# tanqiu98/2G-GCN

Measured on AMD Instinct MI355X. Metric: clips/sec fwd+bwd, T=120 N=34 C=512, higher is better.
Workload: dtype fp32

## Files before the change

2g-gcn_amd/csrc/gemm_f32.hip:

```cpp
#include <cstdlib>
#include "twog_common.h"

typedef float f32x16 __attribute__((ext_vector_type(16)));
typedef float f32x4 __attribute__((ext_vector_type(4)));

namespace {

constexpr int BK = 32;
constexpr int MAXP = 8;

struct Prob {
    twog_rows_t A, B, C;
    const float* bias;
    int M, N, K;
    int act, accumulate;
    int tiles_m, tiles_n, tile_start;
    int a_vec, b_vec;
    int n_major;
    int batch;
    int64_t a_bs, b_bs, c_bs;
    float* cs;
    int cs_acc;
};

// ... 1278 lines not shown
__global__ __launch_bounds__(256, 2) void gemm_ks32_kernel(const Group g) {
    gemm_tile<32, 64, 256, false, BKM, D, false, false, 2>(g, nullptr);
}
template <int D>
__global__ __launch_bounds__(256, 2) void gemm_gate_bwd_ks32_kernel(const Group g, const GateArgs ga) {
    gemm_tile<32, 64, 256, false, true, D, false, true, 2>(g, &ga);
}

template <int BM, int BN>
__global__ __launch_bounds__(256) void splitk_reduce_kernel(const Group g) {
    int bid = blockIdx.x;
    int pi = 0;
#pragma unroll 1
    for (int i = 1; i < g.n; ++i)
        if (bid >= g.p[i].tile_start) pi = i;
    const Prob& P = g.p[pi];
    int tile = bid - P.tile_start;
    const int per_batch = P.tiles_m * P.tiles_n, bi = tile / per_batch;
    tile -= bi * per_batch;
    twog_rows_t C = P.C;
    C.ptr += bi * P.c_bs;
    int tm_idx, tn_idx;
    tile_coords(P, tile, g.group, tm_idx, tn_idx);
    const int m0 = tm_idx * BM, n0 = tn_idx * BN;
    if (P.cs && tn_idx == 0 && blockIdx.y == gridDim.y - 1 && threadIdx.x < 128 && m0 + (int)threadIdx.x < P.M) {
        float v = 0.f;
        for (int s = 0; s < g.splitk; ++s) v += g.cs_part[((int64_t)s * g.total_tiles + bid) * 128 + threadIdx.x];
        float* o = P.cs + m0 + threadIdx.x;
        *o = P.cs_acc ? *o + v : v;
    }
    const int chunk = (BM * BN) / gridDim.y;
    const bool vec = (P.N % 4 == 0) && (reinterpret_cast<uintptr_t>(C.ptr) % 16 == 0) && (C.ld_outer % 4 == 0) &&
                     (C.inner <= 1 || C.ld_inner % 4 == 0) && (!P.bias || reinterpret_cast<uintptr_t>(P.bias) % 16 == 0);
    if (vec) {
        for (int e = blockIdx.y * chunk + threadIdx.x * 4; e < (blockIdx.y + 1) * chunk; e += 1024) {
            const int row = e / BN, col = e - row * BN;
            if (m0 + row >= P.M || n0 + col >= P.N) continue;
            f32x4 v = {0.f, 0.f, 0.f, 0.f};
            for (int s = 0; s < g.splitk; ++s)
                v += *reinterpret_cast<const f32x4*>(g.slabs + ((int64_t)s * g.total_tiles + bid) * (BM * BN) + e);
            float* c = C.ptr + twog_row_off(C, m0 + row) + n0 + col;
            if (P.bias) v += *reinterpret_cast<const f32x4*>(P.bias + n0 + col);
            if (P.accumulate) v += *reinterpret_cast<const f32x4*>(c);
            if (P.act == 1) { v.x = fmaxf(v.x, 0.f); v.y = fmaxf(v.y, 0.f); v.z = fmaxf(v.z, 0.f); v.w = fmaxf(v.w, 0.f); }
            *reinterpret_cast<f32x4*>(c) = v;
        }
        return;
    }
    for (int e = blockIdx.y * chunk + threadIdx.x; e < (blockIdx.y + 1) * chunk; e += 256) {
        const int row = e / BN, col = e - row * BN;
        if (m0 + row >= P.M || n0 + col >= P.N) continue;
        float v = 0.f;
        for (int s = 0; s < g.splitk; ++s) v += g.slabs[((int64_t)s * g.total_tiles + bid) * (BM * BN) + e];
        float* c = C.ptr + twog_row_off(C, m0 + row) + n0 + col;
        if (P.bias) v += P.bias[n0 + col];
        if (P.accumulate) v += *c;
        if (P.act == 1) v = fmaxf(v, 0.f);
        *c = v;
    }
}

inline int vec_ok(const twog_rows_t& m, int64_t batch_stride, int contiguous_extent, int64_t n_rows) {
    const int64_t groups = m.inner > 1 ? (n_rows + m.inner - 1) / m.inner : n_rows;
    const int64_t extent = groups * (m.ld_outer < 0 ? -m.ld_outer : m.ld_outer) + (m.inner > 1 ? (int64_t)m.inner * m.ld_inner : 0);
    if (extent >= (int64_t(1) << 30)) return 0;
    const bool aligned = (reinterpret_cast<uintptr_t>(m.ptr) % 16) == 0;
    const bool ld_ok = (m.ld_outer % 4 == 0) && (m.inner <= 1 || m.ld_inner % 4 == 0) && (batch_stride % 4 == 0);
    return (aligned && ld_ok && contiguous_extent >= 4 && contiguous_extent % 4 == 0) ? 1 : 0;
}

thread_local int g_last_class_x3 = 0;
thread_local int g_precision = TWOG_GEMM_PRECISION_HIGHEST;

template <int NP>
static void launch_x3_128(const Group& g, bool akm, bool bkm, bool kg, dim3 grid, dim3 block, hipStream_t st) {
    if (!akm && !bkm) hipLaunchKernelGGL((gemm_x3_kernel<false, false, false, NP>), grid, block, 0, st, g);
    else if (!akm && bkm && !kg) hipLaunchKernelGGL((gemm_x3_kernel<false, true, false, NP>), grid, block, 0, st, g);
    else if (!akm && bkm) hipLaunchKernelGGL((gemm_x3_kernel<false, true, true, NP>), grid, block, 0, st, g);
    else if (akm && bkm && !kg) hipLaunchKernelGGL((gemm_x3_kernel<true, true, false, NP>), grid, block, 0, st, g);
    else if (akm && bkm) hipLaunchKernelGGL((gemm_x3_kernel<true, true, true, NP>), grid, block, 0, st, g);
    else if (!kg) hipLaunchKernelGGL((gemm_x3_kernel<true, false, false, NP>), grid, block, 0, st, g);
    else hipLaunchKernelGGL((gemm_x3_kernel<true, false, true, NP>), grid, block, 0, st, g);
}

static bool x3_128_ok(const Group& g) {
    static const int x3_on = getenv("TWOG_GEMM_X3") ? atoi(getenv("TWOG_GEMM_X3")) : 1;
    bool ok = x3_on != 0 && (g.k_per_split % X3_BK) == 0;
    for (int i = 0; i < g.n; ++i) ok = ok && g.p[i].a_vec && g.p[i].b_vec && (g.p[i].K % X3_BK) == 0 && g.p[i].M >= 4 && g.p[i].N >= 4;
    return ok;
}

template <int BM, int BN, int NT, int D>
int launch(Group& g, int akm, int bkm, hipStream_t st) {
    g_last_class_x3 = 0;
    dim3 grid(g.total_tiles, g.splitk), block(NT);
    bool kg = false;
    for (int i = 0; i < g.n; ++i) kg = kg || (akm && g.p[i].A.inner > 1) || (bkm && g.p[i].B.inner > 1);
    if constexpr (BM == 128 && NT == 512) {
        if (x3_128_ok(g)) {
            static const int split_acc = getenv("TWOG_X3_DW_SPLIT_ACC") ? atoi(getenv("TWOG_X3_DW_SPLIT_ACC")) : 0;
            const int np = (akm && bkm && split_acc) ? 3 : g_precision == TWOG_GEMM_PRECISION_HIGH ? 2 : g_precision == TWOG_GEMM_PRECISION_MEDIUM ? 1 : 3;
            if (np == 2) launch_x3_128<2>(g, akm, bkm, kg, grid, block, st);
            else if (np == 1) launch_x3_128<1>(g, akm, bkm, kg, grid, block, st);
            else if (!akm && !bkm) hipLaunchKernelGGL((gemm_x3_kernel<false, false, false>), grid, block, 0, st, g);
            else if (!akm && bkm && !kg) hipLaunchKernelGGL((gemm_x3_kernel<false, true, false>), grid, block, 0, st, g);
            else if (!akm && bkm) hipLaunchKernelGGL((gemm_x3_kernel<false, true, true>), grid, block, 0, st, g);
            else if (akm && bkm && split_acc && !kg) hipLaunchKernelGGL((gemm_x3_tt_split_acc_kernel<false>), grid, block, 0, st, g);
            else if (akm && bkm && split_acc) hipLaunchKernelGGL((gemm_x3_tt_split_acc_kernel<true>), grid, block, 0, st, g);
            else if (akm && bkm && !kg) hipLaunchKernelGGL((gemm_x3_kernel<true, true, false>), grid, block, 0, st, g);
            else if (akm && bkm) hipLaunchKernelGGL((gemm_x3_kernel<true, true, true>), grid, block, 0, st, g);
            else if (!kg) hipLaunchKernelGGL((gemm_x3_kernel<true, false, false>), grid, block, 0, st, g);
            else hipLaunchKernelGGL((gemm_x3_kernel<true, false, true>), grid, block, 0, st, g);
            TWOG_CHECK_LAUNCH();
            g_last_class_x3 = np;
            if (g.splitk > 1) {
                hipLaunchKernelGGL((splitk_reduce_kernel<BM, BN>), dim3(g.total_tiles, (BM * BN) / 1024), dim3(256), 0, st, g);
                TWOG_CHECK_LAUNCH();
            }
            return 0;
        }
        if (kg) return launch<BM, BN, 256, D>(g, akm, bkm, st);
    }
    if (!akm && !bkm) hipLaunchKernelGGL((gemm_kernel<BM, BN, NT, false, false, D, false>), grid, block, 0, st, g);
    else if (!akm && bkm && !kg) hipLaunchKernelGGL((gemm_kernel<BM, BN, NT, false, true, D, false>), grid, block, 0, st, g);
    else if (!akm && bkm) hipLaunchKernelGGL((gemm_kernel<BM, BN, NT, false, true, D, true>), grid, block, 0, st, g);
    else if (akm && bkm && !kg) hipLaunchKernelGGL((gemm_kernel<BM, BN, NT, true, true, D, false>), grid, block, 0, st, g);
    else if (akm && bkm) hipLaunchKernelGGL((gemm_kernel<BM, BN, NT, true, true, D, true>), grid, block, 0, st, g);
    else if (!kg) hipLaunchKernelGGL((gemm_kernel<BM, BN, NT, true, false, D, false>), grid, block, 0, st, g);
    else hipLaunchKernelGGL((gemm_kernel<BM, BN, NT, true, false, D, true>), grid, block, 0, st, g);
    TWOG_CHECK_LAUNCH();
    if (g.splitk > 1) {
        hipLaunchKernelGGL((splitk_reduce_kernel<BM, BN>), dim3(g.total_tiles, (BM * BN) / 1024), dim3(256), 0, st, g);
        TWOG_CHECK_LAUNCH();
    }
    return 0;
}

thread_local int g_last_class = 0;

}

extern "C" int twog_gemm_last_class(void) { return g_last_class; }

extern "C" int twog_gemm_set_precision(int p) {
    if (p != TWOG_GEMM_PRECISION_HIGHEST && p != TWOG_GEMM_PRECISION_HIGH && p != TWOG_GEMM_PRECISION_MEDIUM) return -1;
    const int prev = g_precision;
    g_precision = p;
    return prev;
}
extern "C" int twog_gemm_get_precision(void) { return g_precision; }

constexpr size_t SPLITK_TICKET_BYTES = 16384;

static void prepare_group(const twog_gemm_t* pr, int n, int a_kmajor, int b_kmajor, void* workspace,
                          size_t workspace_bytes, Group& g, int* order, bool& big, int& bm) {
    int64_t tiles128 = 0;
    int kmax = 0;
    bool wide = true;
    for (int i = 0; i < n; ++i) {
        const int nb = pr[i].batch > 0 ? pr[i].batch : 1;
        tiles128 += (int64_t)nb * ((pr[i].M + 127) / 128) * ((pr[i].N + 127) / 128);
        if (pr[i].K > kmax) kmax = pr[i].K;
        if (pr[i].M < 96 || pr[i].N < 96) wide = false;
    }
    static const int force_tile = getenv("TWOG_GEMM_TILE") ? atoi(getenv("TWOG_GEMM_TILE")) : 0;
    static const int force_split = getenv("TWOG_GEMM_SPLITK") ? atoi(getenv("TWOG_GEMM_SPLITK")) : 0;
    const int64_t reach128 = tiles128 * (workspace ? (kmax >= 1024 ? kmax / 512 : 1) : 1);
    static const int big_min = getenv("TWOG_GEMM_BIG_MIN") ? atoi(getenv("TWOG_GEMM_BIG_MIN")) : 200;
    big = wide && (tiles128 >= big_min || reach128 >= 256);
    if (force_tile == 128) big = true;
    if (force_tile == 64) big = false;
    const int BMN = big ? 128 : 64;
    bm = BMN;
    {
        static const int bm32_on = getenv("TWOG_GEMM_BM32") ? atoi(getenv("TWOG_GEMM_BM32")) : 1;
        static const int ks_allowed = getenv("TWOG_GEMM_KS") ? atoi(getenv("TWOG_GEMM_KS")) : 1;
        int64_t tiles32 = 0;
        bool plain = true;
        for (int i = 0; i < n; ++i) {
            tiles32 += (int64_t)((pr[i].M + 31) / 32) * ((pr[i].N + 63) / 64);
            plain = plain && pr[i].batch <= 1 && !(b_kmajor && pr[i].B.inner > 1);
        }
        if (bm32_on && ks_allowed && !big && !a_kmajor && !workspace && plain && kmax >= 256 && tiles32 <= 256) bm = 32;
    }
    g.n = n;
    for (int i = 0; i < n; ++i) order[i] = i;
    for (int i = 1; i < n; ++i)
        for (int j = i; j > 0 && pr[order[j]].K > pr[order[j - 1]].K; --j) { const int tmp = order[j]; order[j] = order[j - 1]; order[j - 1] = tmp; }
    int t = 0;
    g.n_cls = 0;
    for (int i = 0; i < n; ++i) {
        Prob& P = g.p[i];
        const twog_gemm_t& q = pr[order[i]];
        P.A = q.A; P.B = q.B; P.C = q.C; P.bias = q.bias;
        P.M = q.M; P.N = q.N; P.K = q.K;
        P.act = q.act; P.accumulate = q.accumulate;
        P.cs = q.a_colsum; P.cs_acc = q.a_colsum_accumulate;
        P.tiles_m = (P.M + bm - 1) / bm;
        P.tiles_n = (P.N + BMN - 1) / BMN;
        P.tile_start = t;
        P.batch = q.batch > 0 ? q.batch : 1;
        static const int force_nmajor = getenv("TWOG_GEMM_NMAJOR") ? atoi(getenv("TWOG_GEMM_NMAJOR")) : -1;
        P.n_major = force_nmajor >= 0 ? force_nmajor : (P.N > P.M ? 1 : 0);
        P.a_bs = q.a_batch_stride; P.b_bs = q.b_batch_stride; P.c_bs = q.c_batch_stride;
        const int ntiles = P.batch * P.tiles_m * P.tiles_n;
        if (i == 0 || P.K != g.p[i - 1].K) {
            g.cls_start[g.n_cls] = t;
            g.cls_ntiles[g.n_cls] = 0;
            ++g.n_cls;
        }
        g.cls_ntiles[g.n_cls - 1] += ntiles;
        t += ntiles;
        P.a_vec = vec_ok(P.A, q.a_batch_stride, a_kmajor ? P.M : P.K, a_kmajor ? P.K : P.M);
        P.b_vec = vec_ok(P.B, q.b_batch_stride, b_kmajor ? P.N : P.K, b_kmajor ? P.K : P.N);
    }
    for (int c = 0, rot = 0; c < g.n_cls; ++c) {
        g.cls_rot[c] = rot & 7;
        rot += g.cls_ntiles[c] & 7;
    }
    g.total_tiles = t;
    static const int group = getenv("TWOG_GEMM_GROUP") ? atoi(getenv("TWOG_GEMM_GROUP")) : 8;
    static const int group64 = getenv("TWOG_GEMM_GROUP64") ? atoi(getenv("TWOG_GEMM_GROUP64")) : 0;
    g.group = big ? group : group64;
    g.splitk = 1;
    g.k_per_split = ((kmax + BK - 1) / BK) * BK;
    g.slabs = nullptr;
    g.cs_part = nullptr;
    g.xcnt = nullptr;
    g.xs_early = 0;
    g.xcd_split = 0;
    if (t < 4096 && kmax >= 1024 && workspace) {
        const int slots = big ? 512 : 1024;
        const int max_by_k = kmax / 256;
        int want = 1;
        double best = 0.0;
        const int max_split = t < 384 ? 64 : 16;
        for (int sft = 1; sft <= max_split && sft <= max_by_k; ++sft) {
            const int64_t wg = (int64_t)t * sft;
            if (wg > (t < 384 ? 2 : 8) * slots && sft > 1) break;
            const double eff = (double)wg / (double)(((wg + slots - 1) / slots) * slots);
            if (eff > best + 0.03) { best = eff; want = sft; }
        }
        if (force_split > 0) want = force_split;
        static const int xcd_on = getenv("TWOG_GEMM_XCD_SPLIT") ? atoi(getenv("TWOG_GEMM_XCD_SPLIT")) : 1;
        int want8 = 0;
        if (xcd_on && big && want > 1 && force_split <= 0 && t <= 512) {
            double best8 = 0.0;
            for (int s8 = 8; s8 <= 64 && s8 <= kmax / 1024; s8 += 8) {
                if ((size_t)s8 * t * BMN * BMN * sizeof(float) + SPLITK_TICKET_BYTES > workspace_bytes) break;
                const int64_t per_xcd = (int64_t)t * s8 / 8;
                const double e8 = (double)per_xcd / (double)(((per_xcd + 63) / 64) * 64);
                if (e8 > best8 + 1e-9) { best8 = e8; want8 = s8; }
                if (e8 >= 0.95) break;
            }
            if (want8 && best8 + 0.08 < best) want8 = 0;
        }
        if (want8) want = want8;
        bool any_cs = false;
        for (int i = 0; i < n; ++i) any_cs = any_cs || pr[i].a_colsum != nullptr;
        const size_t cs_bytes = any_cs ? (size_t)(want + 1) * t * 128 * sizeof(float) : 0;
        const size_t need = (size_t)want * t * BMN * BMN * sizeof(float) + SPLITK_TICKET_BYTES + cs_bytes;
        if (want > 1 && need <= workspace_bytes) {
            int kps = (kmax + want - 1) / want;
            g.k_per_split = ((kps + BK - 1) / BK) * BK;
            g.splitk = (kmax + g.k_per_split - 1) / g.k_per_split;
            g.slabs = reinterpret_cast<float*>(static_cast<char*>(workspace) + SPLITK_TICKET_BYTES);
            g.xcd_split = (want8 && g.splitk % 8 == 0) ? 1 : 0;
            if (any_cs) g.cs_part = g.slabs + (size_t)g.splitk * t * BMN * BMN;
        }
    }
}

static bool x3s_ok(const Group& g, int a_kmajor, int xk, int min_tiles = 96) {
    static const int on = (getenv("TWOG_GEMM_X3") ? atoi(getenv("TWOG_GEMM_X3")) : 1) && (getenv("TWOG_GEMM_X3S") ? atoi(getenv("TWOG_GEMM_X3S")) : 1);
    if (!on || a_kmajor || g.splitk != 1 || g.total_tiles < min_tiles) return false;
    int kmax = 0;
    for (int i = 0; i < g.n; ++i) {
        const Prob& P = g.p[i];
        if (!P.a_vec || !P.b_vec || P.K % xk || P.batch > 1 || P.B.inner > 1 || P.M < 1 || P.N < 4) return false;
        kmax = P.K > kmax ? P.K : kmax;
    }
    return kmax >= 256;
}

static int x3s_ku(const Group& g, int depth) {
    static const int ku = getenv("TWOG_X3S_KU") ? atoi(getenv("TWOG_X3S_KU")) : 2;
    if (ku <= 1) return 1;
    for (int i = 0; i < g.n; ++i)
        if (g.p[i].K % depth) return 1;
    return ku;
}

constexpr size_t XS_COUNTER_BYTES = 16384;
static int pick_xsplit(int tiles, int kmax, int bm, size_t ws_bytes) {
    static const int force = getenv("TWOG_GEMM_XSPLIT") ? atoi(getenv("TWOG_GEMM_XSPLIT")) : 0;
    if (force == 1 || tiles <= 0 || tiles > 4096 || ws_bytes <= XS_COUNTER_BYTES) return 1;
    const int kt = (kmax + BK - 1) / BK;
    const size_t tile_bytes = (size_t)bm * 64 * sizeof(float);
    const int by_ws = (int)((ws_bytes - XS_COUNTER_BYTES) / (tile_bytes * (size_t)tiles));
    if (bm == 32 && force <= 1) {
        int S = kt / 4 < 8 ? kt / 4 : 8;
        while (S > 1 && (tiles * S > 512 || S > by_ws)) --S;
        return S < 1 ? 1 : S;
    }
    const double unit = bm == 32 ? 0.25 : 0.49;
    auto cost = [&](int S) {
        const int per_cu = (tiles * S + 255) / 256, kts = (kt + S - 1) / S;
        return per_cu * kts * unit + (S > 1 ? 3.0 + 0.35 * S : 0.0);
    };
    int best = 1;
    double best_c = cost(1);
    static const int cand[] = {2, 3, 4, 6, 8, 12, 16};
    for (int S : cand) {
        if (S > by_ws || kt / S < 2) break;
        const double c = force > 1 ? (S == force ? -1.0 : 1e30) : cost(S);
        if (c < best_c - 2.5) { best_c = c; best = S; }
    }
    return best;
}

template <class LaunchFn>
static bool try_xsplit(Group& g, int bm, int kmax, void* chain_ws, size_t chain_ws_bytes, LaunchFn launch_fn) {
    if (!chain_ws) return false;
    const int S = pick_xsplit(g.total_tiles, kmax, bm, chain_ws_bytes);
    if (S <= 1) return false;
    const int kt = (kmax + BK - 1) / BK;
    g.k_per_split = ((kt + S - 1) / S) * BK;
    g.splitk = (kmax + g.k_per_split - 1) / g.k_per_split;
    if (g.splitk <= 1) { g.splitk = 1; g.k_per_split = kt * BK; return false; }
    g.xcnt = reinterpret_cast<unsigned*>(chain_ws);
    g.slabs = reinterpret_cast<float*>(reinterpret_cast<char*>(chain_ws) + XS_COUNTER_BYTES);
    static const int early_tiles = getenv("TWOG_GEMM_XS_EARLY") ? atoi(getenv("TWOG_GEMM_XS_EARLY")) : 96;
    g.xs_early = g.total_tiles <= early_tiles ? 1 : 0;
    launch_fn(dim3(g.total_tiles, g.splitk));
    return true;
}

static int pick_xl_split(int tiles, int kmax, size_t ws_bytes) {
    static const int force = getenv("TWOG_X3_XL") ? atoi(getenv("TWOG_X3_XL")) : 0;
    if (force == 1 || tiles < 96 || tiles > 4096 || ws_bytes <= XS_COUNTER_BYTES || kmax % 32) return 1;
    const int kt = kmax / 32;
    const int by_ws = (int)((ws_bytes - XS_COUNTER_BYTES) / ((size_t)64 * 64 * sizeof(float) * (size_t)tiles));
    auto cost = [&](int S) {
        const int r = (tiles * S + 255) / 256;
        return r * ((kt + S - 1) / S) + (S > 1 ? 3 + r : 0);
    };
    int best = 1;
    int best_c = cost(1);
    static const int min_gain = getenv("TWOG_X3_XL_GAIN") ? atoi(getenv("TWOG_X3_XL_GAIN")) : 15;
    static const int cand[] = {2, 3, 4};
    for (int S : cand) {
        if (S > by_ws || kt / S < 8) break;
        const int c = force > 1 ? (S == force ? -1 : (1 << 20)) : cost(S);
        if (c * 100 <= best_c * (100 - min_gain)) { best_c = c; best = S; }
    }
    return best;
}
static bool xl_setup(Group& g, int kmax, void* chain_ws, size_t chain_ws_bytes) {
    if (!chain_ws) return false;
    const int S = pick_xl_split(g.total_tiles, kmax, chain_ws_bytes);
    if (S <= 1) return false;
    const int kt = kmax / 32;
    g.k_per_split = ((kt + S - 1) / S) * 32;
    g.splitk = (kmax + g.k_per_split - 1) / g.k_per_split;
    if (g.splitk <= 1) { g.splitk = 1; g.k_per_split = ((kmax + BK - 1) / BK) * BK; return false; }
    g.xcnt = reinterpret_cast<unsigned*>(chain_ws);
    g.slabs = reinterpret_cast<float*>(reinterpret_cast<char*>(chain_ws) + XS_COUNTER_BYTES);
    g.xcd_split = 0;
    return true;
}

static bool colsums_served(const twog_gemm_t* pr, int n, int a_kmajor, int b_kmajor, const Group& g, bool big) {
    bool any = false, plain = true;
    for (int i = 0; i < n; ++i) {
        any = any || pr[i].a_colsum != nullptr;
        plain = plain && pr[i].batch <= 1 && pr[i].M % 4 == 0 && pr[i].A.inner <= 1 && pr[i].B.inner <= 1;
    }
    if (!any) return true;
    static const int w8 = getenv("TWOG_GEMM_W8") ? atoi(getenv("TWOG_GEMM_W8")) : 1;
    return a_kmajor && b_kmajor && big && w8 && plain && x3_128_ok(g);
}

static bool rows128_pays(const Group& g) {
    static const int on = getenv("TWOG_X3_ROWS128") ? atoi(getenv("TWOG_X3_ROWS128")) : 1;
    if (!on) return false;
    int t64 = 0, t128 = 0;
    for (int i = 0; i < g.n; ++i) {
        const Prob& P = g.p[i];
        if (P.M < 128 || P.batch > 1) return false;
        t64 += ((P.M + 63) / 64) * P.tiles_n;
        t128 += ((P.M + 127) / 128) * P.tiles_n;
    }
    if (t128 < 128 || t128 > 256) return false;
    const int c64 = ((t64 + 255) / 256) * 128, c128 = ((t128 + 255) / 256) * 192;
    return c128 * 100 <= c64 * 85;
}
static void retile_rows(Group& g, int bm) {
    int t = 0;
    g.n_cls = 0;
    for (int i = 0; i < g.n; ++i) {
        Prob& P = g.p[i];
        P.tiles_m = (P.M + bm - 1) / bm;
        P.tile_start = t;
        const int ntiles = P.batch * P.tiles_m * P.tiles_n;
        if (i == 0 || P.K != g.p[i - 1].K) {
            g.cls_start[g.n_cls] = t;
            g.cls_ntiles[g.n_cls] = 0;
            ++g.n_cls;
        }
        g.cls_ntiles[g.n_cls - 1] += ntiles;
        t += ntiles;
    }
    for (int c = 0, rot = 0; c < g.n_cls; ++c) {
        g.cls_rot[c] = rot & 7;
        rot += g.cls_ntiles[c] & 7;
    }
    g.total_tiles = t;
}

static int gemm_impl(const twog_gemm_t* problems, int n_problems, int a_kmajor, int b_kmajor, void* workspace,
                     size_t workspace_bytes, void* chain_ws, size_t chain_ws_bytes, void* stream);

extern "C" int twog_gemm_colsum_fused(const twog_gemm_t* problems, int n_problems, int a_kmajor, int b_kmajor, void* workspace,
                                      size_t workspace_bytes) {
    for (int done = 0; done < n_problems; done += MAXP) {
        const int n = (n_problems - done) < MAXP ? (n_problems - done) : MAXP;
        Group g;
        int order[MAXP];
        bool big;
        int bm;
        prepare_group(problems + done, n, a_kmajor, b_kmajor, workspace, workspace_bytes, g, order, big, bm);
        if (!colsums_served(problems + done, n, a_kmajor, b_kmajor, g, big)) return 0;
    }
    return 1;
}

extern "C" int twog_gemm_f32(const twog_gemm_t* problems, int n_problems, int a_kmajor, int b_kmajor, void* workspace,
                             size_t workspace_bytes, void* stream) {
    return gemm_impl(problems, n_problems, a_kmajor, b_kmajor, workspace, workspace_bytes, nullptr, 0, stream);
}

extern "C" int twog_gemm_f32_chain(const twog_gemm_t* problems, int n_problems, int a_kmajor, int b_kmajor, void* chain_ws,
                                   size_t chain_ws_bytes, void* stream) {
    return gemm_impl(problems, n_problems, a_kmajor, b_kmajor, nullptr, 0, chain_ws, chain_ws_bytes, stream);
}

extern "C" size_t twog_chain_workspace_bytes(void) {
    return XS_COUNTER_BYTES + (size_t)48 * 1024 * 1024;
}

static int gemm_impl(const twog_gemm_t* problems, int n_problems, int a_kmajor, int b_kmajor, void* workspace,
                     size_t workspace_bytes, void* chain_ws, size_t chain_ws_bytes, void* stream) {
    if (n_problems <= 0) return 0;
    hipStream_t st = reinterpret_cast<hipStream_t>(stream);
    {
        bool any_cs = false;
        for (int i = 0; i < n_problems; ++i) any_cs = any_cs || problems[i].a_colsum != nullptr;
        if (any_cs && (chain_ws || !twog_gemm_colsum_fused(problems, n_problems, a_kmajor, b_kmajor, workspace, workspace_bytes))) return -5;
    }
    int done = 0;
    while (done < n_problems) {
        const int n = (n_problems - done) < MAXP ? (n_problems - done) : MAXP;
        const twog_gemm_t* pr = problems + done;
        Group g;
        int order[MAXP];
        bool big;
        int bm;
        prepare_group(pr, n, a_kmajor, b_kmajor, workspace, workspace_bytes, g, order, big, bm);
        static const int depth = getenv("TWOG_GEMM_DEPTH") ? atoi(getenv("TWOG_GEMM_DEPTH")) : 0;
        const int d128 = depth ? (depth & 3) : 2, d64 = depth ? ((depth >> 2) & 3) : 2;
        int rc;
        static const int w8 = getenv("TWOG_GEMM_W8") ? atoi(getenv("TWOG_GEMM_W8")) : 1;
        bool grouped = false;
        for (int i = 0; i < n; ++i) grouped = grouped || (a_kmajor && pr[i].A.inner > 1) || (b_kmajor && pr[i].B.inner > 1);
        g_last_class = (big ? TWOG_GEMM_CLASS_TILE128 : 0) | (big && w8 && !grouped ? TWOG_GEMM_CLASS_WAVES8 : 0) |
                       (grouped ? TWOG_GEMM_CLASS_KG : 0) | (g.splitk > 1 ? TWOG_GEMM_CLASS_SPLITK : 0);
        static const int ks_on = getenv("TWOG_GEMM_KS") ? atoi(getenv("TWOG_GEMM_KS")) : 1;
        int kmax_ = 0;
        for (int i = 0; i < n; ++i) kmax_ = pr[i].K > kmax_ ? pr[i].K : kmax_;
        const bool ks = ks_on && !big && !a_kmajor && !grouped && g.splitk == 1 && g.total_tiles <= 384 && kmax_ >= 256;
        if (!big && bm == 64 && !grouped && chain_ws && x3s_ok(g, a_kmajor, 32) && rows128_pays(g)) {
            retile_rows(g, 128);
            g_last_class |= TWOG_GEMM_CLASS_X3 | TWOG_GEMM_CLASS_WAVES8;
            dim3 grid(g.total_tiles, 1), block(512);
            if (b_kmajor) hipLaunchKernelGGL((gemm_x3su128_kernel<true>), grid, block, 0, st, g);
            else hipLaunchKernelGGL((gemm_x3su128_kernel<false>), grid, block, 0, st, g);
            TWOG_CHECK_LAUNCH();
            done += n;
            continue;
        }
        if (!big && bm == 64 && !grouped && chain_ws && x3s_ok(g, a_kmajor, 32) && xl_setup(g, kmax_, chain_ws, chain_ws_bytes)) {
            g_last_class |= TWOG_GEMM_CLASS_X3 | TWOG_GEMM_CLASS_XSPLIT;
            dim3 grid(g.total_tiles, g.splitk), block(256);
            if (b_kmajor) hipLaunchKernelGGL((gemm_x3su_kernel<true, 1, 2>), grid, block, 0, st, g);
            else hipLaunchKernelGGL((gemm_x3su_kernel<false, 1, 2>), grid, block, 0, st, g);
            TWOG_CHECK_LAUNCH();
            done += n;
            continue;
        }
        if (bm == 32) {
            g_last_class |= TWOG_GEMM_CLASS_KSPLIT | TWOG_GEMM_CLASS_ROWS32;
            if (try_xsplit(g, 32, kmax_, chain_ws, chain_ws_bytes, [&](dim3 grid) {
                    if (b_kmajor) hipLaunchKernelGGL((gemm_xs32_kernel<true, 2>), grid, dim3(256), 0, st, g);
                    else hipLaunchKernelGGL((gemm_xs32_kernel<false, 2>), grid, dim3(256), 0, st, g);
                })) {
                g_last_class |= TWOG_GEMM_CLASS_XSPLIT;
                TWOG_CHECK_LAUNCH();
                done += n;
                continue;
            }
            dim3 grid(g.total_tiles, 1), block(256);
            if (b_kmajor) hipLaunchKernelGGL((gemm_ks32_kernel<true, 2>), grid, block, 0, st, g);
            else hipLaunchKernelGGL((gemm_ks32_kernel<false, 2>), grid, block, 0, st, g);
            TWOG_CHECK_LAUNCH();
            done += n;
            continue;
        }
        if (ks) {
            g_last_class |= TWOG_GEMM_CLASS_KSPLIT;
            if (try_xsplit(g, 64, kmax_, chain_ws, chain_ws_bytes, [&](dim3 grid) {
                    if (b_kmajor) hipLaunchKernelGGL((gemm_xs_kernel<true, 2>), grid, dim3(512), 0, st, g);
                    else hipLaunchKernelGGL((gemm_xs_kernel<false, 2>), grid, dim3(512), 0, st, g);
                })) {
                g_last_class |= TWOG_GEMM_CLASS_XSPLIT;
                TWOG_CHECK_LAUNCH();
                done += n;
                continue;
            }
            dim3 grid(g.total_tiles, 1), block(512);
            if (x3s_ok(g, a_kmajor, 32)) {
                g_last_class |= TWOG_GEMM_CLASS_X3;
                if (g.total_tiles <= 256 && x3s_ku(g, 64) == 2) {
                    if (b_kmajor) hipLaunchKernelGGL((gemm_x3su_kernel<true, 2, 2>), grid, block, 0, st, g);
                    else hipLaunchKernelGGL((gemm_x3su_kernel<false, 2, 2>), grid, block, 0, st, g);
                } else if (b_kmajor) hipLaunchKernelGGL((gemm_x3s_kernel<true, 2>), grid, block, 0, st, g);
                else hipLaunchKernelGGL((gemm_x3s_kernel<false, 2>), grid, block, 0, st, g);
            } else if (b_kmajor) hipLaunchKernelGGL((gemm_ks_kernel<true, 2>), grid, block, 0, st, g);
            else hipLaunchKernelGGL((gemm_ks_kernel<false, 2>), grid, block, 0, st, g);
            TWOG_CHECK_LAUNCH();
            done += n;
            continue;
        }
        static const int x3_try = getenv("TWOG_GEMM_X3") ? atoi(getenv("TWOG_GEMM_X3")) : 1;
        if (big && w8 && (!grouped || x3_try)) rc = d128 == 2 ? launch<128, 128, 512, 2>(g, a_kmajor, b_kmajor, st) : launch<128, 128, 512, 1>(g, a_kmajor, b_kmajor, st);
        else if (big) rc = d128 == 2 ? launch<128, 128, 256, 2>(g, a_kmajor, b_kmajor, st) : launch<128, 128, 256, 1>(g, a_kmajor, b_kmajor, st);
        else if (!big && x3s_ok(g, a_kmajor, 16)) {
            g_last_class |= TWOG_GEMM_CLASS_X3;
            dim3 grid(g.total_tiles, 1), block(256);
            if (x3s_ku(g, 32) == 2) {
                if (b_kmajor) hipLaunchKernelGGL((gemm_x3su_kernel<true, 1, 2>), grid, block, 0, st, g);
                else hipLaunchKernelGGL((gemm_x3su_kernel<false, 1, 2>), grid, block, 0, st, g);
            } else if (b_kmajor) hipLaunchKernelGGL((gemm_x3s_kernel<true, 1>), grid, block, 0, st, g);
            else hipLaunchKernelGGL((gemm_x3s_kernel<false, 1>), grid, block, 0, st, g);
            TWOG_CHECK_LAUNCH();
            rc = 0;
        }
        else rc = d64 == 2 ? launch<64, 64, 256, 2>(g, a_kmajor, b_kmajor, st) : launch<64, 64, 256, 1>(g, a_kmajor, b_kmajor, st);
        if (rc) return rc;
        if (g_last_class_x3) g_last_class |= TWOG_GEMM_CLASS_X3 | TWOG_GEMM_CLASS_WAVES8 |
                                             (g_last_class_x3 == 2 ? TWOG_GEMM_CLASS_P3 : g_last_class_x3 == 1 ? TWOG_GEMM_CLASS_P1 : 0);
        done += n;
    }
    return 0;
}


int twog_internal_gemm_gate_bwd(const twog_gemm_t* pr, int n, const twog_gru_step_bwd_t* gates, float* const* du_part,
                                int dry_run, void* chain_ws, size_t chain_ws_bytes, void* stream) {
    if (n <= 0 || n > MAXP) return 1;
    Group g;
    int order[MAXP];
    bool big;
    int bm;
    prepare_group(pr, n, 0, 1, nullptr, 0, g, order, big, bm);
    if (big || g.splitk != 1) return 1;
    auto span31 = [](const twog_rows_t& m, int rows, int64_t width) {
        const int inner = m.inner > 1 ? m.inner : 1;
        const int64_t last = (int64_t)((rows - 1) / inner) * m.ld_outer + (int64_t)((rows - 1) % inner) * (m.inner > 1 ? m.ld_inner : 0) + width;
        return m.ld_outer >= 0 && m.ld_inner >= 0 && last < (int64_t(1) << 31);
    };
    for (int i = 0; i < n; ++i) {
        if (pr[i].B.inner > 1 || pr[i].batch > 1 || pr[i].bias || pr[i].act) return 1;
        const twog_gru_step_bwd_t& G = gates[i];
        if (G.rows <= 0) continue;
        if ((pr[i].N + 63) / 64 > 8 || G.rows != pr[i].M || G.hidden != pr[i].N || G.rows >= (1 << 22)) return 1;
        const int inner = G.dh.inner > 1 ? G.dh.inner : 1;
        auto same = [&](const twog_rows_t& m) { return (m.inner > 1 ? m.inner : 1) == inner; };
        if (!same(G.save) || !same(G.dgi) || !same(G.dgh) || (G.h_prev.ptr && !same(G.h_prev))) return 1;
        if (G.u && (G.u_inner > 1 ? G.u_inner : 1) != inner) return 1;
        if (G.dh_prev.inner > 1 || G.dh_prev.ptr != pr[i].C.ptr || G.dh_prev_accumulate) return 1;
        const int H3 = 3 * G.hidden;
        if (!span31(G.dh, G.rows, G.hidden) || !span31(G.save, G.rows, 4 * G.hidden) || !span31(G.dgi, G.rows, H3) ||
            !span31(G.dgh, G.rows, H3) || !span31(G.dh_prev, G.rows, G.hidden) ||
            (G.h_prev.ptr && !span31(G.h_prev, G.rows, G.hidden)))
            return 1;
        if (G.u && ((int64_t)((G.rows - 1) / inner) * G.u_ld_outer + (int64_t)((G.rows - 1) % inner) * G.u_ld_inner >= (int64_t(1) << 31)))
            return 1;
    }
    if (dry_run) return 0;
    GateArgs ga;
    for (int i = 0; i < n; ++i) {
        const int src = order[i];
        ga.gate_of[i] = gates[src].rows > 0 ? i : -1;
        ga.s[i] = gates[src];
        ga.du_part[i] = (gates[src].rows > 0 && gates[src].du && du_part) ? du_part[src] : nullptr;
    }
    for (int i = n; i < MAXP; ++i) { ga.gate_of[i] = -1; ga.du_part[i] = nullptr; }
    static const int depth = getenv("TWOG_GEMM_DEPTH") ? atoi(getenv("TWOG_GEMM_DEPTH")) : 0;
    const int d64 = depth ? ((depth >> 2) & 3) : 2;
    dim3 grid(g.total_tiles, 1), block(256);
    g_last_class = TWOG_GEMM_CLASS_GATE;
    static const int ks_on = getenv("TWOG_GEMM_KS") ? atoi(getenv("TWOG_GEMM_KS")) : 1;
    int kmax = 0;
    for (int i = 0; i < n; ++i) kmax = pr[i].K > kmax ? pr[i].K : kmax;
    if (bm == 64 && chain_ws && x3s_ok(g, 0, 32) && xl_setup(g, kmax, chain_ws, chain_ws_bytes)) {
        g_last_class |= TWOG_GEMM_CLASS_X3 | TWOG_GEMM_CLASS_XSPLIT;
        hipLaunchKernelGGL((gemm_gate_bwd_x3su_kernel<1, 2>), dim3(g.total_tiles, g.splitk), dim3(256), 0, (hipStream_t)stream, g, ga);
        TWOG_CHECK_LAUNCH();
        return 0;
    }
    if (bm == 32) {
// ... 127 lines not shown
```

2g-gcn_amd/ops.py:

```python
import contextlib
import math
import os
import weakref

import torch

from .kernels import get_kernels

SUPPORTED_NOTE = ("the HIP path implements every constructor configuration of the reference's TGGCN: message_type "
                  "'v1' (relational) / 'v2', message_granularity 'v1' / 'v2', aggregation 'att' / 'mp', attention_style "
                  "'v1'..'v4', distance-based attention, every gate strategy and position feature. Sender-only messages "
                  "with dot-product attention or mean pooling (every configuration shipped in the reference's "
                  "conf/models/) run on the tuned kernels (attn.hip, segrnn.hip), the other forms on the general "
                  "single-relation kernels (relation.hip)")


def _v2(t, width=None):
    return t.view(-1, t.shape[-1] if width is None else width)


class Plan:

    def __init__(self, cfg, bs, T, H, O, N, F_o, n_sub, n_aff, human_seg_given, object_seg_given):
        h = cfg['hidden_size']
# ... 119 lines not shown
            'sh': 'geometry_to_human_message_att_mlp', 'so': 'geometry_to_object_message_att_mlp'}
_REL_ENDS = {'hh': ('h', 'h'), 'oh': ('h', 'o'), 'sh': ('h', 's'), 'ho': ('o', 'h'), 'so': ('o', 's'), 'oo': ('o', 'o')}


def _head_name(plan, name):
    return name.replace('_frame', '') if plan.share_heads else name


def used_parameter_names(plan: Plan):
    g = 'geometry_embedding_gcn.'
    names = [g + 'joint_embed.cnn.0.bn.weight', g + 'joint_embed.cnn.0.bn.bias',
             g + 'joint_embed.cnn.1.cnn.weight', g + 'joint_embed.cnn.1.cnn.bias',
             g + 'joint_embed.cnn.3.cnn.weight', g + 'joint_embed.cnn.3.cnn.bias',
             g + 'get_s.s1.cnn.weight', g + 'get_s.s1.cnn.bias', g + 'get_s.s2.cnn.weight', g + 'get_s.s2.cnn.bias',
             g + 'weight']
    for m in ('geometry_embedding_mlp.0', 'geometry_embedding_mlp.2', 'human_embedding_mlp.0',
              'object_embedding_mlp.0', 'human_bd_embedding_mlp.0', 'object_bd_embedding_mlp.0',
              'geometry_bd_embedding_mlp.0'):
        names += [m + '.weight', m + '.bias']
    for r in ('human_bd_rnn', 'object_bd_rnn', 'geometry_bd_rnn'):
        for sfx in ('', '_reverse'):
            names += [f'{r}.weight_ih_l0{sfx}', f'{r}.weight_hh_l0{sfx}', f'{r}.bias_ih_l0{sfx}', f'{r}.bias_hh_l0{sfx}']
    for rel in plan.snd_h + plan.snd_o + plan.snd_s:
        if plan.relational:
            names += [f'{_REL_PREFIX[rel]}_{kind}_relation_mlp.0.{wb}' for kind in ('pairwise', 'full')
                      for wb in ('weight', 'bias')]
        else:
            names += [_FRAME_MLP[rel] + '.0.weight', _FRAME_MLP[rel] + '.0.bias']
            if not plan.mean_pool and plan.att_style != 'dot':
                names += [_ATT_MLP[rel] + ('.weight' if plan.att_style == 'general' else '.0.weight'),
                          _ATT_MLP[rel] + ('.bias' if plan.att_style == 'general' else '.0.bias')]
    if plan.msg_segment:
        for rel in ('hh', 'ho', 'oh', 'oo'):
            if not getattr(plan, 'rel_' + rel):
                continue
            if plan.relational:
                names += [f'{_REL_PREFIX[rel]}_segment_{kind}_relation_mlp.0.{wb}' for kind in ('pairwise', 'full')
                          for wb in ('weight', 'bias')]
                continue
            names += [_SEG_MLP[rel] + '.0.weight', _SEG_MLP[rel] + '.0.bias']
            if not plan.mean_pool and plan.att_style != 'dot':
                a_ = _ATT_MLP[rel].replace('_message_att_mlp', '_segment_message_att_mlp')
                names += [a_ + ('.weight' if plan.att_style == 'general' else '.0.weight'),
                          a_ + ('.bias' if plan.att_style == 'general' else '.0.bias')]
    for cell in ('human_segment_rnn_fcell', 'human_segment_rnn_bcell', 'object_segment_rnn_fcell',
                 'object_segment_rnn_bcell'):
        names += [cell + '.weight_ih', cell + '.weight_hh', cell + '.bias_ih', cell + '.bias_hh']
    for on, mlp in ((plan.learn_h, 'update_human_segment_mlp'), (plan.own_o, 'update_object_segment_mlp')):
        if on:
            for layer in range(plan.n_gate_hidden + 1):
                names += [f'{mlp}.{2 * layer}.weight', f'{mlp}.{2 * layer}.bias']
    if not plan.periodic:
        if plan.time_s or plan.time_u:
            names += ['time_position_mlp.0.weight', 'time_position_mlp.0.bias']
        if plan.seglen:
            names += ['segment_length_mlp.0.weight', 'segment_length_mlp.0.bias']
    heads = ['human_frame_recognition_mlp', 'human_frame_prediction_mlp', 'human_recognition_mlp',
             'human_prediction_mlp']
    if plan.n_aff is not None:
        heads += ['object_frame_recognition_mlp', 'object_frame_prediction_mlp', 'object_recognition_mlp',
                  'object_prediction_mlp']
    for m in heads:
        m = _head_name(plan, m)
        names += [m + '.0.weight', m + '.0.bias']
    if not plan.has_bias:
        names = [n for n in names if n.startswith('geometry_embedding_gcn.') or
                 not (n.endswith('.bias') or '.bias_' in n)]
    seen, out = set(), []
    for n in names:
        if n not in seen:
            seen.add(n)
            out.append(n)
    return out


_MODEL_EXTRAS = weakref.WeakKeyDictionary()


def set_model_extra(model, key, value):
    d = _MODEL_EXTRAS.setdefault(model, {})
    if value is None:
        d.pop(key, None)
    else:
        d[key] = value


def get_model_extra(model, key):
    return _MODEL_EXTRAS.get(model, {}).get(key)


def set_grad_stage_hook(model, fn):
    set_model_extra(model, 'stage_hook', fn)


def pack_weights(K, groups):
    out, pairs = {}, []
    for key, tensors in groups.items():
        if not tensors:
            out[key] = None
            continue
        t0 = tensors[0]
        buf = torch.empty((sum(t.shape[0] for t in tensors),) + tuple(t0.shape[1:]), dtype=torch.float32, device=t0.device)
        r = 0
        for t in tensors:
            src = t.detach()
            pairs.append((src if src.is_contiguous() else src.contiguous(), buf[r:r + t.shape[0]]))
            r += t.shape[0]
        out[key] = buf
    K.copy_blocks(pairs)
    return out


def grad_ready_stage(name: str) -> int:
    if ('_segment_rnn_' in name or name.startswith('update_') or 'recognition_mlp' in name or 'prediction_mlp' in name
            or any(name.startswith(v) for v in _SEG_MLP.values())):
        return 0
    if '_bd_rnn' in name or '_bd_embedding_mlp' in name or any(name.startswith(v) for v in _FRAME_MLP.values()):
        return 1
    return 2


def enable_grad_sinks(params, on: bool = True):
    for p in params:
        p._twog_grad_sink = bool(on)


def _stage_done(plan, stage, G=None):
    if G is not None:
        G.flush()
    hook = getattr(plan, 'stage_hook', None)
    if isinstance(hook, weakref.WeakMethod):
        hook = hook()
    if hook is not None:
        hook(stage)


class _Params(dict):

    def __missing__(self, k):
        if k.endswith('.bias') or '.bias_' in k:
            return None
        raise KeyError(k)


class _Grads:

    def __init__(self, K, sinks=None, known=None):
        self.K, self.g, self.sinks, self.known = K, {}, sinks or {}, known
        self._pending, self._pending_dst = [], set()
        self._pend_cs, self._pend_cp = [], []
        self._pend_mm_wide = True
        self._pend_mm, self._pend_mm_c = [], set()
        self._held = None
        self._defer = hasattr(K, 'colsum_many') and os.environ.get('TWOG_BATCH_ADDS', '1') != '0'
        self._verify = os.environ.get('TWOG_VERIFY_DEFERRED', '0') == '1'
        self._snaps = []

    def _snap(self, *tensors):
        if not self._verify:
            return
        outs = [q['C'] for q in self._pend_mm] + [o for _, _, o, _ in self._pend_cs] + [d for _, d in self._pend_cp]
        if self._held is not None:
            outs += [self._held['C']] + ([self._held['colsum']] if self._held.get('colsum') is not None else [])
        pending = {o.untyped_storage().data_ptr() for o in outs}
        self._snaps += [(t, t.detach().clone()) for t in tensors
                        if t is not None and t.untyped_storage().data_ptr() not in pending]

    def _check_snaps(self):
        snaps, self._snaps = self._snaps, []
        for t, was in snaps:
            if not torch.equal(t, was):
                raise RuntimeError('an operand of a deferred gradient launch changed between the call and flush() '
                                   f'(shape {tuple(t.shape)}): the deferred form would have computed a different gradient')

    def sink(self, name):
        return self.sinks.get(name)

    def has(self, name):
        return self.known is None or dict.__contains__(self.known, name)

    def add(self, name, t):
        if not self.has(name):
            return
        dst = self.sinks.get(name)
        if dst is None:
            dst = self.g.get(name)
        if dst is not None:
            if not hasattr(self.K, 'rowops') or os.environ.get('TWOG_BATCH_ADDS', '1') == '0':
                self.K.add_rows(_v2(t.reshape(1, -1)), _v2(dst.view(1, -1)))
                return
            key = dst.data_ptr()
            if key in self._pending_dst or len(self._pending) >= 16:
                self.flush()
            self._pending.append(('add', _v2(t.reshape(1, -1)), _v2(dst.view(1, -1))))
            self._pending_dst.add(key)
            self._snap(t)
        else:
            self.g[name] = t

    def dw_gemm(self, problem):
        A, B = problem['A'], problem['B']

        def plain(t):
            n = t.shape[0] if t.dim() == 2 else t.shape[0] * t.shape[1]
            return (t.shape[-1] % 4 == 0 and t.data_ptr() % 16 == 0 and all(st % 4 == 0 for st in t.stride()[:-1]) and n % 16 == 0)

        rows = A.shape[0] if A.dim() == 2 else A.shape[0] * A.shape[1]
        wide = A.shape[-1] >= 128 and B.shape[-1] >= 128 and rows <= 8192 and plain(A) and plain(B)
        narrow = ((A.shape[-1] < 128 or B.shape[-1] < 128) and 0 < rows <= int(os.environ.get('TWOG_BATCH_DW_NARROW_ROWS', '20000')))
        if narrow and self._holdable(problem):
            narrow = False
        if not self._defer or os.environ.get('TWOG_BATCH_DW', '1') == '0' or not (wide or narrow):
            self._issue_held()
            if problem['C'].data_ptr() in self._pend_mm_c:
                self.flush()
            if self._holdable(problem):
                self._held = problem
                self._snap(A, B)
                return
            self.K.gemm([problem], a_kmajor=True, b_kmajor=True)
            return
        key = problem['C'].data_ptr()
        if key in self._pend_mm_c or len(self._pend_mm) >= 8 or (self._pend_mm and self._pend_mm_wide != wide):
            self.flush()
        self._pend_mm.append(problem)
        self._pend_mm_c.add(key)
        self._pend_mm_wide = wide
        self._snap(A, B)

    def _holdable(self, problem):
        return (self._defer and problem['A'].dim() == 2 and os.environ.get('TWOG_DW_COLSUM', '1') != '0'
                and hasattr(self.K, 'gemm_colsum_ok') and self.K.gemm_colsum_ok(problem))

    def colsum(self, x, out=None, accumulate=False):
        if out is None:
            out, accumulate = torch.empty(x.shape[-1], dtype=torch.float32, device=x.device), False
        if not self._defer:
            return self.K.colsum(x, out=out, accumulate=accumulate)
        h = self._held
        if h is not None:
            A = h['A']
            if (A.data_ptr() == x.data_ptr() and A.shape == x.shape and A.stride() == x.stride() and out.is_contiguous()
                    and not any(o.data_ptr() == out.data_ptr() for _, _, o, _ in self._pend_cs)):
                h['colsum'], h['colsum_accumulate'] = out, accumulate
            self._issue_held()
            if 'colsum' in h:
                return out
        if len(self._pend_cs) >= 16 or any(o.data_ptr() == out.data_ptr() for _, _, o, _ in self._pend_cs):
            self.flush()
        self._pend_cs.append((x, None, out, accumulate))
        self._snap(x)
        return out

    def copy(self, src, dst):
        if not self._defer:
            dst.copy_(src)
            return
        self._pend_cp.append((src, dst))

    def _issue_held(self):
        h, self._held = self._held, None
        if h is not None:
            if self._verify and not self._pend_mm and not self._pend_cs and not self._pending:
                self._check_snaps()
            self.K.gemm([h], a_kmajor=True, b_kmajor=True)

    def flush(self):
        if self._verify:
            self._check_snaps()
        self._issue_held()
        if self._pend_mm:
            self.K.gemm(self._pend_mm, a_kmajor=True, b_kmajor=True)
            self._pend_mm, self._pend_mm_c = [], set()
        if self._pend_cs:
            self.K.colsum_many(self._pend_cs)
            self._pend_cs = []
        if self._pend_cp:
            self.K.copy_blocks(self._pend_cp)
            self._pend_cp = []
        if self._pending:
            self.K.rowops(self._pending)
            self._pending, self._pending_dst = [], set()


def _gru_bias_grads(K, G, b_ih, b_hh, dgi, dgh, h):
    if not (G.has(b_ih) or G.has(b_hh)):
        return
    db_ih = G.colsum(dgi)
    if G.has(b_hh):
        db_hh = torch.empty(3 * h, dtype=torch.float32, device=dgi.device)
        G.copy(db_ih[:2 * h], db_hh[:2 * h])
        G.colsum(dgh[:, 2 * h:], out=db_hh[2 * h:])
        G.add(b_hh, db_hh)
    G.add(b_ih, db_ih)


def _lin_w_grads(K, G, wname, bname, dY, X, cols=None, total=None):
    N, Kin = dY.shape[-1], X.shape[-1]
    dst = G.sink(wname)
    if cols is not None:
        c0, c1 = cols
        if dst is None:
            dst = G.g.get(wname)
            if dst is None:
                dst = torch.zeros(N, total, dtype=torch.float32, device=dY.device)
                G.g[wname] = dst
        G.dw_gemm(dict(A=dY, B=X, C=dst.view(N, total)[:, c0:c1], accumulate=True))
    elif dst is not None:
        G.dw_gemm(dict(A=dY, B=X, C=dst.view(N, Kin), accumulate=True))
    else:
        dW = torch.empty(N, Kin, dtype=torch.float32, device=dY.device)
        G.dw_gemm(dict(A=dY, B=X, C=dW))
        G.add(wname, dW)
    _bias_grad(K, G, bname, dY)


def geo_gcn_forward(K, P, x_human, bs, T, N, training, bn_bufs, S, save_x=True):
    dev, nF = x_human.device, bs * T

    def empty(*shape):
        return torch.empty(*shape, dtype=torch.float32, device=dev)

    g = 'geometry_embedding_gcn.'
    wq, wk = P[g + 'get_s.s1.cnn.weight'].view(128, 64), P[g + 'get_s.s2.cnn.weight'].view(128, 64)
    ab, mi, md = K.bn_fold(x_human, N, P[g + 'joint_embed.cnn.0.bn.weight'], P[g + 'joint_embed.cnn.0.bn.bias'],
                           bn_bufs['running_mean'], bn_bufs['running_var'], bn_bufs['num_batches_tracked'], training,
                           stats_reduce=bn_bufs.get('stats_reduce'), fold=(wq, wk, P[g + 'get_s.s1.cnn.bias']))
    w1 = P[g + 'joint_embed.cnn.1.cnn.weight'].view(64, 4)
    w2 = P[g + 'joint_embed.cnn.3.cnn.weight'].view(64, 64)
    X, adj, Z = K.gcn_fused_fwd(x_human, N, ab, w1, P[g + 'joint_embed.cnn.1.cnn.bias'], w2,
                                P[g + 'joint_embed.cnn.3.cnn.bias'], md, save_x=save_x)
    Gout = empty(bs, 128, N, T)
    Zv = Z.view(bs, T, N, 64).permute(0, 2, 1, 3)
    K.gemm([dict(A=P[g + 'weight'], B=Zv[0], C=Gout[0].view(128, N * T), batch=(bs, 0, T * N * 64, 128 * N * T))],
           a_kmajor=True, b_kmajor=False)
    S.update(ab=ab, mi=mi, X=X, md=md, adj=adj, Z=Z)
    return Gout


def _rel_distance_view(p, dists, rel, n_inst):
    d = dists or {}
    H, O = p.H, p.O
    if rel == 'hh' and d.get('hh') is not None:
        return d['hh'].reshape(n_inst, H, H)
    if rel == 'oh' and d.get('ho') is not None:
        return d['ho'].reshape(n_inst, H, O)
    if rel == 'ho' and d.get('ho') is not None:
        return d['ho'].reshape(n_inst, H, O).transpose(1, 2)
    if rel == 'oo' and d.get('oo') is not None:
        return d['oo'].reshape(n_inst, O, O)
    return None


class _RelLevel:

    def __init__(self, p, segment, n_inst, ipc, feats, outs, dists, scale, dfeats=None, douts=None):
        self.p, self.segment, self.n_inst, self.ipc = p, segment, n_inst, ipc
        self.feats, self.outs, self.dists, self.scale = feats, outs, dists, scale
        self.dfeats, self.douts = dfeats, douts
        self.D = p.h if segment else 2 * p.h
        self.sizes = {'h': p.H, 'o': p.O, 's': 1}

    def names(self, rel):
        seg = '_segment' if self.segment else ''
        msg = (_SEG_MLP if self.segment else _FRAME_MLP)[rel] + '.0'
        att = _ATT_MLP[rel].replace('_message_att_mlp', seg + '_message_att_mlp')
        return dict(msg=msg, att=att, g=f'{_REL_PREFIX[rel]}{seg}_pairwise_relation_mlp.0',
                    f=f'{_REL_PREFIX[rel]}{seg}_full_relation_mlp.0')

    def recv_masked(self, rel):
        return (not self.segment) and rel in ('ho', 'so')


class _Staged:

    def __init__(self, K):
        self.K = K
        self._gemm, self._rf, self._rb, self._ops = {}, [], [], []

    def gemm(self, problems, **flags):
        self._gemm.setdefault(tuple(sorted(flags.items())), []).extend(problems)

    def relation_fwd(self, f):
        self._rf.append(f)

    def relation_bwd(self, b):
        self._rb.append(b)

    def relu_bwd(self, dy, y, dx):
        self._ops.append(('relu_bwd', dy, y, dx))

    def rank1_update(self, dst, s_, v):
        self._ops.append(('rank1', dst, s_, v))

    @staticmethod
    def _waves(items, targets):
        waves = []
        for it in items:
            t = targets(it)
            for w_items, w_t in waves:
                if not (t & w_t):
                    w_items.append(it)
                    w_t |= t
                    break
            else:
                waves.append(([it], set(t)))
        return [w for w, _ in waves]

    @staticmethod
    def _rb_targets(b):
        return {b[k].data_ptr() for k, acc in (('dq', 'dq_accumulate'), ('dk', 'dk_accumulate'))
                if b.get(acc) and b.get(k) is not None}

    def flush(self):
        K = self.K
        for flags, probs in self._gemm.items():
            for wave in self._waves(probs, lambda g: {g['C'].data_ptr()} if g.get('accumulate') else set()):
                K.gemm(wave, **dict(flags))
        if self._rf:
            K.relation_fwd_many(self._rf)
        for wave in self._waves(self._rb, self._rb_targets):
            K.relation_bwd_many(wave)
        for wave in self._waves(self._ops, lambda o: {o[1].data_ptr()} if o[0] == 'rank1' else set()):
# ... 1411 lines not shown
```

Before: 964.5.

## Group tall-K weight-gradient GEMMs sharing an input into one XCD-split launch

Weight-gradient GEMMs with many rows (very large K) that share the same A operand are now deferred on the Python side and issued together as one grouped GEMM. The C++ side detects these tall groups, forces 128-wide tiles and an XCD-aligned split-K, and orders problems so that ones sharing A sit next to each other. If no split can be chosen it falls back to issuing each problem separately. The aim is fewer small launches and better use of all compute units for these large-K reductions. The cost is more deferral bookkeeping and extra workspace for the split-K slabs.

```diff
diff --git a/2g-gcn_amd/csrc/gemm_f32.hip b/2g-gcn_amd/csrc/gemm_f32.hip
--- a/2g-gcn_amd/csrc/gemm_f32.hip
+++ b/2g-gcn_amd/csrc/gemm_f32.hip
@@ -1454,6 +1454,19 @@
 
 constexpr size_t SPLITK_TICKET_BYTES = 16384;
 
+constexpr int TALL_GROUP_MIN_K = 8192;
+static bool tall_group(const twog_gemm_t* pr, int n, int a_kmajor, int b_kmajor, const void* workspace) {
+    static const int on = getenv("TWOG_GEMM_TALL_GROUPS") ? atoi(getenv("TWOG_GEMM_TALL_GROUPS")) : 1;
+    static const int forced = (getenv("TWOG_GEMM_TILE") ? atoi(getenv("TWOG_GEMM_TILE")) : 0) || (getenv("TWOG_GEMM_SPLITK") ? atoi(getenv("TWOG_GEMM_SPLITK")) : 0);
+    if (!on || forced || n < 2 || !a_kmajor || !b_kmajor || !workspace || pr[0].K < TALL_GROUP_MIN_K) return false;
+    int64_t tiles = 0;
+    for (int i = 0; i < n; ++i) {
+        if (pr[i].K != pr[0].K || pr[i].batch > 1 || pr[i].M < 96 || pr[i].N < 96) return false;
+        tiles += (int64_t)((pr[i].M + 127) / 128) * ((pr[i].N + 127) / 128);
+    }
+    return tiles < 4096;
+}
+
 static void prepare_group(const twog_gemm_t* pr, int n, int a_kmajor, int b_kmajor, void* workspace,
                           size_t workspace_bytes, Group& g, int* order, bool& big, int& bm) {
     int64_t tiles128 = 0;
@@ -1470,6 +1483,8 @@
     const int64_t reach128 = tiles128 * (workspace ? (kmax >= 1024 ? kmax / 512 : 1) : 1);
     static const int big_min = getenv("TWOG_GEMM_BIG_MIN") ? atoi(getenv("TWOG_GEMM_BIG_MIN")) : 200;
     big = wide && (tiles128 >= big_min || reach128 >= 256);
+    const bool tall = tall_group(pr, n, a_kmajor, b_kmajor, workspace);
+    if (tall) big = true;
     if (force_tile == 128) big = true;
     if (force_tile == 64) big = false;
     const int BMN = big ? 128 : 64;
@@ -1489,6 +1504,15 @@
     for (int i = 0; i < n; ++i) order[i] = i;
     for (int i = 1; i < n; ++i)
         for (int j = i; j > 0 && pr[order[j]].K > pr[order[j - 1]].K; --j) { const int tmp = order[j]; order[j] = order[j - 1]; order[j - 1] = tmp; }
+    if (tall) {
+        int m = 0;
+        bool placed[MAXP] = {};
+        for (int i = 0; i < n; ++i) {
+            if (placed[i]) continue;
+            for (int j = i; j < n; ++j)
+                if (!placed[j] && pr[j].A.ptr == pr[i].A.ptr) { order[m++] = j; placed[j] = true; }
+        }
+    }
     int t = 0;
     g.n_cls = 0;
     for (int i = 0; i < n; ++i) {
@@ -1546,7 +1570,7 @@
         if (force_split > 0) want = force_split;
         static const int xcd_on = getenv("TWOG_GEMM_XCD_SPLIT") ? atoi(getenv("TWOG_GEMM_XCD_SPLIT")) : 1;
         int want8 = 0;
-        if (xcd_on && big && want > 1 && force_split <= 0 && t <= 512) {
+        if (xcd_on && big && (want > 1 || tall) && force_split <= 0 && (t <= 512 || tall)) {
             double best8 = 0.0;
             for (int s8 = 8; s8 <= 64 && s8 <= kmax / 1024; s8 += 8) {
                 if ((size_t)s8 * t * BMN * BMN * sizeof(float) + SPLITK_TICKET_BYTES > workspace_bytes) break;
@@ -1555,9 +1579,10 @@
                 if (e8 > best8 + 1e-9) { best8 = e8; want8 = s8; }
                 if (e8 >= 0.95) break;
             }
-            if (want8 && best8 + 0.08 < best) want8 = 0;
+            if (!tall && want8 && best8 + 0.08 < best) want8 = 0;
         }
         if (want8) want = want8;
+        else if (tall) want = 1;
         bool any_cs = false;
         for (int i = 0; i < n; ++i) any_cs = any_cs || pr[i].a_colsum != nullptr;
         const size_t cs_bytes = any_cs ? (size_t)(want + 1) * t * 128 * sizeof(float) : 0;
@@ -1732,6 +1757,11 @@
         bool big;
         int bm;
         prepare_group(problems + done, n, a_kmajor, b_kmajor, workspace, workspace_bytes, g, order, big, bm);
+        if (tall_group(problems + done, n, a_kmajor, b_kmajor, workspace) && g.splitk == 1) {
+            for (int i = 0; i < n; ++i)
+                if (problems[done + i].a_colsum && !twog_gemm_colsum_fused(problems + done + i, 1, a_kmajor, b_kmajor, workspace, workspace_bytes)) return 0;
+            continue;
+        }
         if (!colsums_served(problems + done, n, a_kmajor, b_kmajor, g, big)) return 0;
     }
     return 1;
@@ -1769,6 +1799,14 @@
         bool big;
         int bm;
         prepare_group(pr, n, a_kmajor, b_kmajor, workspace, workspace_bytes, g, order, big, bm);
+        if (tall_group(pr, n, a_kmajor, b_kmajor, workspace) && g.splitk == 1) {
+            for (int i = 0; i < n; ++i) {
+                const int rc1 = gemm_impl(pr + i, 1, a_kmajor, b_kmajor, workspace, workspace_bytes, chain_ws, chain_ws_bytes, stream);
+                if (rc1) return rc1;
+            }
+            done += n;
+            continue;
+        }
         static const int depth = getenv("TWOG_GEMM_DEPTH") ? atoi(getenv("TWOG_GEMM_DEPTH")) : 0;
         const int d128 = depth ? (depth & 3) : 2, d64 = depth ? ((depth >> 2) & 3) : 2;
         int rc;
diff --git a/2g-gcn_amd/ops.py b/2g-gcn_amd/ops.py
--- a/2g-gcn_amd/ops.py
+++ b/2g-gcn_amd/ops.py
@@ -295,7 +295,9 @@
         self._pend_mm_wide = True
         self._pend_mm, self._pend_mm_c = [], set()
         self._held = None
+        self._tall, self._tall_c = {}, set()
         self._defer = hasattr(K, 'colsum_many') and os.environ.get('TWOG_BATCH_ADDS', '1') != '0'
+        self._tall_on = self._defer and os.environ.get('TWOG_BATCH_DW_TALL', '1') != '0'
         self._verify = os.environ.get('TWOG_VERIFY_DEFERRED', '0') == '1'
         self._snaps = []
 
@@ -305,6 +307,8 @@
         outs = [q['C'] for q in self._pend_mm] + [o for _, _, o, _ in self._pend_cs] + [d for _, d in self._pend_cp]
         if self._held is not None:
             outs += [self._held['C']] + ([self._held['colsum']] if self._held.get('colsum') is not None else [])
+        for grp in self._tall.values():
+            outs += [q['C'] for q in grp] + [q['colsum'] for q in grp if q.get('colsum') is not None]
         pending = {o.untyped_storage().data_ptr() for o in outs}
         self._snaps += [(t, t.detach().clone()) for t in tensors
                         if t is not None and t.untyped_storage().data_ptr() not in pending]
@@ -357,6 +361,22 @@
             self._issue_held()
             if problem['C'].data_ptr() in self._pend_mm_c:
                 self.flush()
+            if problem['C'].data_ptr() in self._tall_c:
+                self._issue_tall()
+            if self._tall_on and A.shape[-1] >= 128 and B.shape[-1] >= 128 and rows > 8192 and plain(A) and plain(B):
+                key = (A.data_ptr(), tuple(A.shape), tuple(A.stride()))
+                grp = self._tall.get(key)
+                if grp is not None and any(q.get('colsum') is not None for q in grp) and not self._holdable(problem):
+                    self._issue_tall(key)
+                    grp = None
+                if grp is None:
+                    grp = self._tall[key] = []
+                grp.append(problem)
+                self._tall_c.add(problem['C'].data_ptr())
+                self._snap(A, B)
+                if len(grp) >= 8:
+                    self._issue_tall(key)
+                return
             if self._holdable(problem):
                 self._held = problem
                 self._snap(A, B)
@@ -364,6 +384,8 @@
             self.K.gemm([problem], a_kmajor=True, b_kmajor=True)
             return
         key = problem['C'].data_ptr()
+        if key in self._tall_c:
+            self._issue_tall()
         if key in self._pend_mm_c or len(self._pend_mm) >= 8 or (self._pend_mm and self._pend_mm_wide != wide):
             self.flush()
         self._pend_mm.append(problem)
@@ -389,6 +411,14 @@
             self._issue_held()
             if 'colsum' in h:
                 return out
+        grp = self._tall.get((x.data_ptr(), tuple(x.shape), tuple(x.stride()))) if self._tall else None
+        if grp is not None:
+            taken = [o.data_ptr() for _, _, o, _ in self._pend_cs] + [q['colsum'].data_ptr() for g_ in self._tall.values()
+                                                                      for q in g_ if q.get('colsum') is not None]
+            if (out.is_contiguous() and out.data_ptr() not in taken and all(q.get('colsum') is None for q in grp)
+                    and all(self._holdable(q) for q in grp)):
+                grp[0]['colsum'], grp[0]['colsum_accumulate'] = out, accumulate
+                return out
         if len(self._pend_cs) >= 16 or any(o.data_ptr() == out.data_ptr() for _, _, o, _ in self._pend_cs):
             self.flush()
         self._pend_cs.append((x, None, out, accumulate))
@@ -408,10 +438,17 @@
                 self._check_snaps()
             self.K.gemm([h], a_kmajor=True, b_kmajor=True)
 
+    def _issue_tall(self, key=None):
+        for k in ([key] if key is not None else list(self._tall)):
+            self.K.gemm(self._tall.pop(k), a_kmajor=True, b_kmajor=True)
+        self._tall_c = {q['C'].data_ptr() for grp in self._tall.values() for q in grp}
+
     def flush(self):
         if self._verify:
             self._check_snaps()
         self._issue_held()
+        if self._tall:
+            self._issue_tall()
         if self._pend_mm:
             self.K.gemm(self._pend_mm, a_kmajor=True, b_kmajor=True)
             self._pend_mm, self._pend_mm_c = [], set()
```

Measured after the change: 963.8. About the same (-0.1%).
